# HKUST-KnowComp/DualMessagePassing

Hardware: AMD Instinct MI355X
Metric: (pattern,graph) pairs/sec DMPNN fwd+bwd hid=128 (higher is better)
Workload: dtype f32

## Files before the change

dualmessagepassing_amd/_abi.py:

```python
import ctypes

c_int = ctypes.c_int
c_i32 = ctypes.c_int32
c_i64 = ctypes.c_int64
c_u64 = ctypes.c_uint64
c_f32 = ctypes.c_float
c_double = ctypes.c_double
c_ptr = ctypes.c_void_p
c_size = ctypes.c_size_t

ABI_VERSION = 97

DMP_COLLATE_MAX_JOBS = 4
DMP_POOL_MAX_JOBS = 4
DMP_REDUCE_MAX_SEGMENTS = 16
DMP_ADAMW_MAX_SKIP = 16
DMP_ADAMW_MAX_SEGMENTS = 1024
DMP_LOOKUP_MAX_JOBS = 8
DMP_CONCAT_MAX_JOBS = 12
DMP_GEMM_MAX_JOBS = 12
DMP_GEMM_MAX_TERMS = 3
DMP_ATB_MAX_JOBS = 8
DMP_MEM_MEAN, DMP_MEM_SUM, DMP_MEM_MAX = 0, 1, 2
DMP_LRP_MAX_NEIGHBOURS = 32
# ... 197 lines not shown
    "dmp_smallk_atb_blocks": (c_i64, [c_i64]),
    "dmp_smallk_embed_cols": (c_int, [c_ptr, c_i64, c_int, c_ptr, c_i64, c_ptr, c_i64, c_int, c_int, c_ptr, c_i64, c_ptr]),
    "dmp_smallk_atb_cols_masked": (c_int, [c_ptr, c_i64, c_int, c_ptr, c_i64, c_int, c_ptr, c_i64, c_ptr, c_ptr, c_i64, c_int, c_ptr, c_ptr]),
    "dmp_smallk_atb_cols_rows": (c_int, [c_ptr, c_i64, c_int, c_ptr, c_i64, c_int, c_ptr, c_i64, c_ptr, c_ptr, c_i64, c_int, c_ptr, c_ptr]),
    "dmp_smallk_atb": (c_int, [c_ptr, c_i64, c_int, c_ptr, c_i64, c_ptr, c_i64, c_int, c_ptr, c_ptr]),
    "dmp_smallk_atb_jobs": (c_int, [_p(dmp_smallk_job), c_int, c_int, c_int, c_ptr]),
    "dmp_l0_pack_jobs": (c_int, [_p(dmp_l0_pack_job), c_int, c_ptr]),
    "dmp_count_loss": (c_int, [c_ptr, c_ptr, c_i64, c_int, c_f32, c_ptr, c_ptr, c_ptr]),
    "dmp_match_loss_workspace_words": (c_i64, [c_i64, c_i64]),
    "dmp_match_loss": (c_int, [c_ptr, c_i64, c_ptr, c_ptr, c_ptr, c_ptr, c_ptr, c_i64, c_i64, c_int, c_ptr, c_ptr, c_ptr, c_ptr, c_ptr]),
    "dmp_reduce_partials_multi": (c_int, [c_ptr, c_ptr, c_ptr, c_ptr, c_int, c_ptr]),
    "dmp_l0_pack": (c_int, [c_ptr, c_i64, c_i64, c_ptr, c_i64, c_ptr, c_i64, c_int, c_int, c_int, c_ptr, c_ptr]),
    "dmp_l0_edge_fwd_masked": (c_int, [c_ptr, c_i64, c_int, c_ptr, c_i64, c_ptr, c_i64, c_ptr, c_ptr, c_ptr, c_ptr, c_ptr, c_i64, c_int,
                                       c_f32, c_ptr, c_i64, c_ptr]),
    "dmp_l0_bwd_w_blocks": (c_i64, [c_i64]),
    "dmp_l0_node_pack_rows": (c_i64, []),
    "dmp_l0_node_fwd": (c_int, [c_ptr, c_i64, c_int, c_ptr, c_i64, c_int, c_int, c_ptr, c_i64, c_ptr, c_f32, c_ptr,
                                c_ptr, c_ptr, c_i64, c_i64, c_i64, c_i64, c_int, c_ptr, c_i64, c_ptr, c_i64, c_ptr]),
    "dmp_bn_partial_rows": (c_i64, [c_i64, c_int]),
    "dmp_bn_train_fwd": (c_int, [c_ptr, c_i64, c_i64, c_int, c_ptr, c_ptr, c_f32, c_f32, c_ptr, c_ptr, c_int, c_f32, c_ptr, c_ptr, c_ptr,
                                 c_i64, c_ptr]),
    "dmp_bn_train_bwd": (c_int, [c_ptr, c_i64, c_ptr, c_i64, c_ptr, c_i64, c_i64, c_int, c_ptr, c_int, c_f32, c_ptr, c_ptr, c_ptr, c_i64,
                                 c_ptr]),
    "dmp_bn_train_fwd_rows": (c_int, [c_ptr, c_i64, c_i64, c_ptr, c_int, c_ptr, c_ptr, c_f32, c_f32, c_ptr, c_ptr, c_int, c_f32, c_ptr, c_ptr,
                                      c_ptr, c_i64, c_ptr]),
    "dmp_bn_train_bwd_rows": (c_int, [c_ptr, c_i64, c_ptr, c_i64, c_ptr, c_i64, c_i64, c_ptr, c_int, c_ptr, c_int, c_f32, c_ptr, c_ptr, c_ptr,
                                      c_i64, c_ptr]),
    "dmp_l0_bwd_w_masked": (c_int, [c_ptr, c_i64, c_int, c_ptr, c_ptr, c_i64, c_ptr, c_i64, c_ptr, c_i64, c_int, c_ptr, c_ptr]),
    "dmp_scalar_filter_gates": (c_int, [_p(dmp_filter_job), c_int, c_i64, c_ptr, c_i64, c_ptr]),
    "dmp_csr_pair_workspace_words": (c_size, [c_i64]),
    "dmp_csr_build_pair": (c_int, [c_ptr, c_ptr, c_ptr, c_i64, c_i64, c_ptr, c_ptr, c_ptr, c_ptr, c_ptr, c_ptr, c_ptr, c_ptr, c_ptr,
                                   c_ptr, c_ptr]),
    "dmp_heads_blend": (c_int, [c_ptr, c_ptr, c_ptr, c_int, c_int, c_ptr, c_ptr]),
    "dmp_concat_pairs": (c_int, [_p(dmp_concat_job), c_int, c_ptr]),
    "dmp_table_rows": (c_int, [_p(dmp_lookup_job), c_int, c_ptr]),
    "dmp_len_masks": (c_int, [_p(dmp_mask_job), c_int, c_i64, c_ptr]),
    "dmp_pack_segments": (c_int, [c_ptr, c_ptr, c_ptr, c_int, c_int, c_ptr, c_ptr]),
    "dmp_adamw_step": (c_int, [c_ptr, c_ptr, c_ptr, c_ptr, c_ptr, c_i64, c_double, c_double, c_double, c_double,
                               c_double, c_i64, c_ptr]),
    "dmp_adamw_step_skip": (c_int, [c_ptr, c_ptr, c_ptr, c_ptr, c_ptr, c_i64, c_double, c_double, c_double, c_double,
                                    c_double, c_i64, c_ptr, c_ptr, c_int, c_ptr]),
    "dmp_adamw_step_dev": (c_int, [c_ptr, c_ptr, c_ptr, c_ptr, c_ptr, c_i64, c_ptr, c_double, c_double, c_double, c_double,
                                   c_ptr, c_ptr, c_int, c_ptr]),
    "dmp_adamw_step_segments": (c_int, [c_ptr, c_ptr, c_ptr, c_ptr, c_ptr, c_i64, c_ptr, c_ptr, c_int, c_ptr, c_ptr, c_ptr, c_double, c_double,
                                        c_double, c_double, c_ptr, c_int, c_ptr]),
    "dmp_adamw_step_guarded": (c_int, [c_ptr, c_ptr, c_ptr, c_ptr, c_ptr, c_i64, c_ptr, c_double, c_double, c_double, c_double,
                                       c_ptr, c_ptr, c_int, c_ptr, c_int, c_ptr]),
    "dmp_edge_select_build": (c_int, [c_ptr, c_ptr, c_ptr, c_ptr, c_i64, c_ptr, c_ptr, c_ptr, c_ptr]),
    "dmp_edge_select_nodes": (c_int, [c_ptr, c_ptr, c_ptr, c_ptr, c_i64, c_ptr, c_ptr, c_ptr, c_ptr]),
    "dmp_edge_fwd_fused": (c_int, [c_ptr, c_i64, c_ptr, c_i64, c_ptr, c_i64, c_i64, c_ptr, c_ptr, c_ptr, c_ptr,
                                   c_i64, c_int, c_f32, c_ptr, c_i64, c_ptr]),
    "dmp_edge_fwd_typed": (c_int, [c_ptr, c_i64, c_ptr, c_i64, c_ptr, c_i64, c_i64, c_ptr, c_ptr, c_ptr, c_ptr, c_ptr,
                                   c_ptr, c_i64, c_i64, c_int, c_f32, c_ptr, c_i64, c_ptr]),
    "dmp_bwd_z_typed_arow": (c_int, [c_ptr, c_i64, c_ptr, c_i64, c_ptr, c_i64, c_i64, c_ptr, c_i64, c_ptr, c_ptr, c_f32,
                                     c_f32, c_ptr, c_ptr, c_ptr, c_ptr, c_i64, c_i64, c_int, c_int, c_ptr, c_i64, c_ptr, c_i64, c_ptr]),
    "dmp_mask_slots": (c_int, [c_ptr, c_i64, c_ptr, c_i64, c_ptr, c_ptr]),
    "dmp_pool_relu_bwd_blocks": (c_i64, [c_i64, c_int]),
    "dmp_pool_relu_bwd": (c_int, [c_ptr, c_i64, c_ptr, c_i64, c_ptr, c_ptr, c_ptr, c_ptr, c_i64, c_i64, c_int, c_f32, c_ptr, c_i64,
                                  c_ptr, c_ptr, c_ptr]),
    "dmp_relu_bwd_gathered_colsum": (c_int, [c_ptr, c_i64, c_ptr, c_ptr, c_ptr, c_i64, c_i64, c_int, c_f32, c_ptr, c_i64, c_ptr, c_ptr]),
    "dmp_dev_set_exact_fp32": (None, [c_int]),
    "dmp_dev_get_exact_fp32": (c_int, []),
    "dmp_rel_gemm": (c_int, [c_ptr, c_i64, c_i64, c_ptr, c_i64, c_int, c_int, c_ptr, c_ptr, c_ptr, c_ptr, c_i64, c_ptr, c_i64,
                             c_int, c_ptr, c_i64, c_ptr]),
    "dmp_rel_atb_blocks": (c_i64, [c_int]),
    "dmp_rel_atb": (c_int, [c_ptr, c_i64, c_i64, c_ptr, c_i64, c_i64, c_ptr, c_ptr, c_ptr, c_ptr, c_int, c_i64, c_int, c_ptr, c_ptr]),
# ... 107 lines not shown
```

dualmessagepassing_amd/csrc/dmp_heads.hip:

```cpp
#include "dmp_common.h"

namespace dmp {
namespace {

constexpr int kThreads = 256, kRows = 16;
constexpr int kMaxHeads = DMP_HEADS_MAX;

template <int kH> struct HeadGeom {
  static constexpr int kF = 4 * kH + 4, kYS = kH + 4;
  static constexpr int kPad = kH + 4, kFPad = 4 * kH + 8;
  static constexpr int CW = kH / 16;
  static constexpr int NT = kH / 64, NKB = kH / 16;
};

__device__ __forceinline__ float4 ldg4(const float *p) { return *reinterpret_cast<const float4 *>(p); }

struct Heads {
  dmp_head_weights w[kMaxHeads];
  dmp_head_io io[kMaxHeads];
  dmp_head_grads gr[kMaxHeads];
  int B;
  float slope;
};

// ... 285 lines not shown
    if (!ok16p(io[i].ps) || !ok16p(io[i].gs) || !io[i].pl || !io[i].gl || !ok16p(io[i].F) || !ok16p(io[i].Y1S) || !io[i].y ||
        io[i].ld_ps < kH || io[i].ld_gs < kH || io[i].ld_ps % 4 || io[i].ld_gs % 4)
      return false;
  }
  return true;
}

constexpr int kLossThreads = 1024;
__global__ __launch_bounds__(kLossThreads) void count_loss_k(const float *__restrict__ pred, const float *__restrict__ target, int64_t n,
                                                             int kind, float slope, float *__restrict__ loss, float *__restrict__ dpred) {
  __shared__ float red[kLossThreads];
  const float inv_n = 1.f / (float)n;
  float acc = 0.f;
  for (int64_t i = threadIdx.x; i < n; i += kLossThreads) {
    const float p = pred[i];
    const float da = p > 0.f ? 1.f : slope;
    const float d = p * da - target[i];
    float v, g;
    if (kind == 0) { v = d * d; g = 2.f * d; }
    else if (kind == 1) { v = fabsf(d); g = d > 0.f ? 1.f : (d < 0.f ? -1.f : 0.f); }
    else { const float a = fabsf(d); v = a < 1.f ? 0.5f * d * d : a - 0.5f; g = a < 1.f ? d : (d > 0.f ? 1.f : -1.f); }
    acc += v;
    dpred[i] = g * da * inv_n;
  }
  red[threadIdx.x] = acc;
  __syncthreads();
  for (int w = kLossThreads / 2; w > 0; w >>= 1) {
    if ((int)threadIdx.x < w) red[threadIdx.x] += red[threadIdx.x + w];
    __syncthreads();
  }
  if (threadIdx.x == 0) loss[0] = red[0] * inv_n;
}

}
}

using namespace dmp;

extern "C" {

int dmp_heads_forward(const dmp_head_weights *w, const dmp_head_io *io, int num_heads, int B, int H, float slope,
                      void *stream) {
  if ((H != 128 && H != 64 && H > 0) || !slope_ok(slope)) return DMP_ERR_UNSUPPORTED;
  if (!heads_valid(w, io, num_heads, B, H)) return DMP_ERR_BAD_ARG;
  if (B == 0) return DMP_OK;
  Heads t;
  for (int i = 0; i < num_heads; ++i) { t.w[i] = w[i]; t.io[i] = io[i]; t.gr[i] = dmp_head_grads{}; }
  t.B = B; t.slope = slope;
  const dim3 grid((unsigned)((B + kRows - 1) / kRows), (unsigned)num_heads);
  if (H == 128) heads_fwd_k<128><<<grid, kThreads, 0, (hipStream_t)stream>>>(t);
  else heads_fwd_k<64><<<grid, kThreads, 0, (hipStream_t)stream>>>(t);
  return check_launch();
}

int dmp_heads_blend(const float *const *y, const float *const *gl, float *const *w, int num_heads, int B, float *out,
                    void *stream) {
  if (num_heads < 1 || num_heads > kMaxHeads || B < 0 || !y || !gl || !w) return DMP_ERR_BAD_ARG;
  if (B == 0) return DMP_OK;
  if (!out) return DMP_ERR_BAD_ARG;
  BlendArgs a;
  for (int i = 0; i < num_heads; ++i) {
    if (!y[i] || !gl[i] || !w[i]) return DMP_ERR_BAD_ARG;
    a.y[i] = y[i]; a.gl[i] = gl[i]; a.w[i] = w[i];
  }
  a.out = out; a.n = num_heads; a.B = B;
  heads_blend_k<<<(unsigned)((B + kThreads - 1) / kThreads), kThreads, 0, (hipStream_t)stream>>>(a);
// ... 10 lines not shown
        (g[i].dgs && (!ok16p(g[i].dgs) || g[i].ld_dgs % 4)) || !g[i].dWp || !g[i].dbp || !g[i].dWg || !g[i].dbg || !g[i].dW1 ||
        !g[i].db1 || !g[i].dW2 || !g[i].db2)
      return DMP_ERR_BAD_ARG;
  }
  if (B == 0) return DMP_OK;
  Heads t;
  WJobs wj;
  wj.n = 0; wj.B = B;
  int blocks = 0;
  for (int i = 0; i < num_heads; ++i) {
    t.w[i] = w[i]; t.io[i] = io[i]; t.gr[i] = g[i];
    add_wjob(wj, blocks, g[i].dY1, kH, kH, nullptr, io[i].F, kF, kF, g[i].dW1, kF, g[i].db1, 1.0f);
    add_wjob(wj, blocks, g[i].dP, kH, kH, nullptr, io[i].ps, io[i].ld_ps, kH, g[i].dWp, kH, g[i].dbp, io[i].scale_p);
    add_wjob(wj, blocks, g[i].dG, kH, kH, nullptr, io[i].gs, io[i].ld_gs, kH, g[i].dWg, kH, g[i].dbg, io[i].scale_g);
    add_wjob(wj, blocks, g[i].dy, 1, 1, g[i].dy_scale, io[i].Y1S, kYS, kYS, g[i].dW2, kYS, g[i].db2, 1.0f);
  }
  t.B = B; t.slope = slope;
  const dim3 grid((unsigned)((B + kRows - 1) / kRows), (unsigned)num_heads);
  if (H == 128) heads_bwd_rows_k<128><<<grid, kThreads, 0, (hipStream_t)stream>>>(t);
  else heads_bwd_rows_k<64><<<grid, kThreads, 0, (hipStream_t)stream>>>(t);
  int rc = check_launch();
  if (rc != DMP_OK) return rc;
  heads_bwd_w_k<<<(unsigned)blocks, kThreads, 0, (hipStream_t)stream>>>(wj);
  return check_launch();
}

int dmp_count_loss(const float *pred, const float *target, int64_t n, int kind, float neg_slope, float *loss, float *dpred, void *stream) {
  if (n < 1 || kind < 0 || kind > 2 || !pred || !target || !loss || !dpred) return DMP_ERR_BAD_ARG;
  if (n > ((int64_t)1 << 22) || !(neg_slope >= 0.f && neg_slope <= 1.f)) return DMP_ERR_UNSUPPORTED;
  count_loss_k<<<1, kLossThreads, 0, (hipStream_t)stream>>>(pred, target, n, kind, neg_slope, loss, dpred);
  return check_launch();
}

}
```

dualmessagepassing_amd/fused.py:

```python
import ctypes as _ctypes
import os as _os
import threading

import torch
from torch.autograd.function import once_differentiable

from . import _abi, _lib, gatememo, ops, side
from ._lib import check, ptr, stream_ptr


def _partials(rows, H, dev):
    lib = _lib.load()
    return torch.empty((int(lib.dmp_colsum_partial_rows(rows, H)), H), dtype=torch.float32, device=dev)


MAX_REDUCE_SEGMENTS = _abi.DMP_REDUCE_MAX_SEGMENTS


class _Deferred(threading.local):

    def __init__(self):
        self.stack = []


# ... 63 lines not shown
    lib = _lib.load()
    R, H = d_out.shape
    part = _partials(R, H, d_out.device)
    d_upd = torch.empty_like(d_out) if gate is not None else None
    with _lib.timed("scale_rows_colsum[H=%d,R=%d]", (H, R), 4 * H * R * (2 if gate is not None else 1)):
        check(lib.dmp_scale_rows_colsum(ptr(d_out), H, ptr(gate), R, H, ptr(d_upd), H, ptr(part), stream_ptr()),
              "dmp_scale_rows_colsum")
    return (d_upd if gate is not None else d_out), reduce_partials(part)


def relu_bwd_colsum_(d_h, act, out=None, slope=0.0):
    lib = _lib.load()
    R, H = d_h.shape
    part = _partials(R, H, d_h.device)
    dst = d_h if out is None else out
    ldo = dst.stride(0) if R > 1 else H
    with _lib.timed("relu_bwd_colsum[H=%d,R=%d]", (H, R), 12 * H * R):
        check(lib.dmp_relu_bwd_colsum(ptr(d_h), H, ptr(act), H, R, H, slope, ptr(dst), ldo, ptr(part), stream_ptr()),
              "dmp_relu_bwd_colsum")
    return dst, reduce_partials(part)


def relu_bwd_gathered_colsum(table, rowmap, gate, act, slope=0.0):
    lib = _lib.load()
    R, H = act.shape
    part = _partials(R, H, act.device)
    out = torch.empty((R, H), dtype=torch.float32, device=act.device)
    with _lib.timed("relu_bwd_gathered[H=%d,R=%d]", (H, R), 8 * H * R + 8 * R + 4 * H * table.size(0)):
        check(lib.dmp_relu_bwd_gathered_colsum(ptr(table), table.stride(0), ptr(rowmap), ptr(gate), ptr(act), act.stride(0), R, H,
                                               slope, ptr(out), H, ptr(part), stream_ptr()), "dmp_relu_bwd_gathered_colsum")
    return out, reduce_partials(part)


def pool_relu_bwd(table, rowmap, gate, act, pool, slope=0.0, skip_dead=False):
    lib = _lib.load()
    R, H = act.shape
    V = pool.num_chunks
    nb = int(lib.dmp_pool_relu_bwd_blocks(V, H))
    part = torch.empty((nb, H), dtype=torch.float32, device=act.device)
    kc = keep_pool_csr(pool, gate) if skip_dead else None
    vptr, vent = (pool.vptr, pool.vent) if kc is None else kc
    out = dead_rows_buffer((R, H), act.device) if kc is not None else torch.empty((R, H), dtype=torch.float32, device=act.device)
    qc = torch.empty((V, 2 * H), dtype=torch.float32, device=act.device)
    with _lib.timed("pool_relu_bwd[H=%d,R=%d]", (H, R), 8 * H * R + 12 * R + 8 * H * V):
        check(lib.dmp_pool_relu_bwd(ptr(act), act.stride(0), ptr(table), table.stride(0), ptr(rowmap), ptr(gate), ptr(vptr),
                                    ptr(vent), V, R, H, slope, ptr(out), H, ptr(qc), ptr(part), stream_ptr()), "dmp_pool_relu_bwd")
    Q = ops.seg_sum_raw(qc, pool.gptr, pool.gent, pool.num_graphs, None, False, rows_shared=False)
    return out, reduce_partials(part), Q


def keep_pool_csr(pool, gate):
    own = None if gate is None else gatememo.owner(gate)
    if not has_row_mask(own, True, True) or pool.num_chunks == 0 or gate.numel() == 0:
        return None
    return gatememo.memo(own, ("keep_pool", id(pool)), (pool,), lambda: _csr_keep(pool.vptr, pool.vent, gate, pool.num_chunks), True)


def _csr_keep_buffers(rows, entries, device):
    nscr = int(_lib.load().dmp_csr_keep_scratch_words(rows))
    ws = torch.empty(nscr + rows + 1 + entries, dtype=torch.int32, device=device)
    return ws[:nscr], ws[nscr:nscr + rows + 1], ws[nscr + rows + 1:]


def _csr_keep(csr_ptr, csr_ent, gate, rows):
    row_cnt, kptr, kent = _csr_keep_buffers(rows, csr_ent.numel(), csr_ptr.device)
    check(_lib.load().dmp_csr_keep(ptr(csr_ptr), ptr(csr_ent), ptr(gate.reshape(-1)), rows, csr_ent.numel(), ptr(row_cnt), ptr(kptr),
                                   ptr(kent), stream_ptr()), "dmp_csr_keep")
    return kptr, kent


def pool_rows(x, pool, weight=None):
    split = pool.flag8 is not None
    kc = keep_pool_csr(pool, weight) if (weight is not None and x.size(1) % 4 == 0 and x.is_contiguous()) else None
    if kc is not None:
        part = ops.seg_sum_raw(x, kc[0], kc[1], pool.num_chunks, None, split, 1.0, 1.0, rows_shared=False)
    else:
        part = ops.seg_sum_raw(x, pool.vptr, pool.vent, pool.num_chunks, weight, split, 1.0, 1.0, rows_shared=False)
    return ops.seg_sum_raw(part, pool.gptr, pool.gent, pool.num_graphs, None, False, rows_shared=False)


def pool_weight_sums(pool, weight=None):
    lib = _lib.load()
    if not getattr(pool, "rows_in_order", False):
        raise _lib.DmpError("pool_weight_sums: an index over rows in their own order")

    def build():
        halves = 2 if pool.flag8 is not None else 1
        out = torch.empty((pool.num_graphs, halves), dtype=torch.float32, device=pool.offsets.device)
        w = None if weight is None else weight.reshape(-1).contiguous()
        check(lib.dmp_pool_weight_sums(ptr(w), ptr(pool.flag8), ptr(pool.offsets), pool.num_graphs, ptr(out), stream_ptr()),
              "dmp_pool_weight_sums")
        return out

    if weight is None or weight.requires_grad:
        return build()
    return gatememo.memo(weight, "pool_weight_sums", (pool,), build)


def pool_rowmap(pool):
    m = getattr(pool, "_rowmap", None)
    if m is None:
        m = pool.seg32 if pool.flag8 is None else torch.where(pool.flag8 != 0, torch.full_like(pool.seg32, -1), pool.seg32)
        pool._rowmap = m
    return m


def bwd_g_colsum(d_y, coef, dst32):
    lib = _lib.load()
    E, H = d_y.shape
    part = _partials(E, H, d_y.device)
    d_g = torch.empty((E, 2 * H), dtype=torch.float32, device=d_y.device)
# ... 1247 lines not shown
    lib = _lib.load()
    if not 0 < len(jobs) <= _abi.DMP_GEMM_MAX_JOBS:
        raise _lib.DmpError("small_gemm_jobs: 1..%d jobs" % _abi.DMP_GEMM_MAX_JOBS)
    J = (_abi.dmp_gemm_job * len(jobs))()

    def ld(t):
        if t.dim() != 2 or t.dtype != torch.float32 or (t.size(1) > 1 and t.stride(1) != 1):
            raise _lib.DmpError("small_gemm_jobs: 2-D fp32 operands with unit inner stride")
        return t.stride(0) if t.size(0) > 1 else max(t.size(1), 1)

    keep = []
    for n, (out, terms, addend) in enumerate(jobs):
        M, N = out.shape
        if not 0 < len(terms) <= _abi.DMP_GEMM_MAX_TERMS:
            raise _lib.DmpError("small_gemm_jobs: 1..%d terms per job" % _abi.DMP_GEMM_MAX_TERMS)
        _lib.require_gpu(out, addend, *[x for tm in terms for x in (tm[0], tm[2])])
        for q, (A, ta, B, tb) in enumerate(terms):
            K = A.size(0) if ta else A.size(1)
            if (A.size(1) if ta else A.size(0)) != M or (B.size(1) if tb else B.size(0)) != K or (B.size(0) if tb else B.size(1)) != N:
                raise _lib.DmpError("small_gemm_jobs: shapes of job %d, term %d" % (n, q))
            T = J[n].term[q]
            T.A, T.lda, T.B, T.ldb, T.transA, T.transB, T.K = A.data_ptr(), ld(A), B.data_ptr(), ld(B), int(bool(ta)), int(bool(tb)), K
            keep.append((A, B))
        J[n].num_terms, J[n].M, J[n].N, J[n].C, J[n].ldc = len(terms), M, N, out.data_ptr(), ld(out)
        if addend is not None:
            if addend.shape != out.shape:
                raise _lib.DmpError("small_gemm_jobs: addend shape")
            J[n].C0, J[n].ldc0 = addend.data_ptr(), ld(addend)
    check(lib.dmp_small_gemm_jobs(J, len(jobs), stream_ptr()), "dmp_small_gemm_jobs")


class _LayerCall:
    __slots__ = ("index", "coef", "residual", "H", "N", "slope", "inner", "v_gate", "e_gate", "Bn", "bn", "Wx", "Wes", "be",
                 "nW2", "nb2", "eW2", "eb2", "WesT", "nW2t", "eW2t", "l0", "W0", "WV0", "nd", "vpool", "epool")

    def __init__(self, **facts):
        for name in self.__slots__:
            setattr(self, name, facts[name])


def _kept_nodes(index, H, v_gate, l0):
    side.wait("nodes")
    return node_rows(index, v_gate, H) if kept_node_path(index, H, v_gate, l0) else None


def _xn_buffer(c, device):
    return dead_rows_buffer((c.N, c.H), device) if (c.inner & 1) else torch.zeros((c.N, c.H), dtype=torch.float32, device=device)


def _l0_param_products(c, node_pass, device):
    l0, W0, WV0, H, Bn, Wx = c.l0, c.W0, c.WV0, c.H, c.Bn, c.Wx
    K0, TK = l0.K, W0.size(0)
    M0 = torch.empty((TK, 2 * H), dtype=torch.float32, device=device)
    jobs = [(M0, [(W0, False, c.Wes, False)], None)]
    WP = WB = MV = None
    if node_pass:
        VK = l0.VK
        WP = torch.zeros((TK // K0, L0_NODE_MAX_COLS, 3 * H), dtype=torch.float32, device=device)
        for t in range(TK // K0):
            WVt = WV0 if WV0.size(0) == VK else WV0[t * VK:(t + 1) * VK]
            jobs += [(WP[t, :VK], [(WVt, False, Wx, False)], None),
                     (WP[t, VK:VK + K0, :H], [(W0[t * K0:(t + 1) * K0], False, Bn[:H], False)], None),
                     (WP[t, VK + K0:VK + 2 * K0, :H], [(W0[t * K0:(t + 1) * K0], False, Bn[H:], False)], None)]
    else:
        WB = torch.empty((2, TK, H), dtype=torch.float32, device=device)
        jobs += [(WB[0], [(W0, False, Bn[:H], False)], None), (WB[1], [(W0, False, Bn[H:], False)], None)]
        if l0.venc is not None:
# ... 137 lines not shown
        tiles = _edge_out_tiles(c, z, dead, False)
        if tiles is not None:
            H1e = dead_rows_buffer((z.size(0), H), z.device)
            zn = out_fwd_typed(H1e, c.eW2t, c.eb2, z, tiles,
                               first=dict(z=z, Wes=c.Wes, P=P, ldp=ldp, bias=c.be, coef=c.coef, index=c.index, slope=c.slope, sel=sel))
            return H1e, zn
    if typed_ok(c.index, H):
        return edge_fwd_typed(z, c.Wes, P, ldp, c.be, c.coef, c.index, c.slope, dead_gate=dead_gate, sel=sel), None
    G = z @ c.Wes
    H1e = edge_combine_raw(G, 2 * H, P, ldp, c.be, c.coef, c.index, H, relu=True, slope=c.slope)
    del G
    if sums_only:
        return H1e, None
    Oe = torch.addmm(c.eb2, H1e, c.eW2.t())
    return H1e, gate_residual(z if c.residual else None, Oe, c.e_gate)


def _edge_out(c, z, H1e):
    l0 = c.l0
    _, dead = _dead_edge_rows_of(c)
    side.wait("tiles")
    codes = _residual_from_codes(c, H1e)
    tiles = _edge_out_tiles(c, H1e, dead, codes)
    if tiles is None:
        return out_fwd_mfma(H1e, c.eW2, c.eb2, c.e_gate, l0_rows(l0, c.W0, z) if c.residual else None, c.eW2t, dead_rows=dead)
    walk = ascending_tiles(c.e_gate) or tiles
    if codes:
        return out_fwd_typed_codes(H1e, c.eW2t, c.eb2, l0.enc, l0.K, c.W0[-l0.K:], walk, prev=l0.z_head, row0=l0.z_head.size(0))
    return out_fwd_typed(H1e, c.eW2t, c.eb2, l0_rows(l0, c.W0, z) if c.residual else None, walk)


def _pooled_outputs(c, z, xn, zn, H1e, sums_only):
    H, epool, e_gate, eW2, eb2 = c.H, c.epool, c.e_gate, c.eW2, c.eb2
    vs = pool_rows(xn, c.vpool) if c.vpool is not None else None
    if not sums_only:
        return vs, (pool_rows(zn, epool) if epool is not None else None), None
    halves = 2 if epool.flag8 is not None else 1
    G_ = epool.num_graphs
    Q = pool_rows(H1e, epool, e_gate).view(G_ * halves, H)
    gcnt = pool_weight_sums(epool, e_gate)
    cnt = gcnt.view(G_ * halves, 1)
    zs = pool_rows(z, epool, e_gate if zero_rows_gate(e_gate) else None).view(G_ * halves, H) if c.residual else None
    if Q.is_contiguous() and eW2.is_contiguous() and Q.size(0) <= SMALL_GEMM_MAX_ROWS:
        es = torch.empty((G_ * halves, H), dtype=torch.float32, device=Q.device)
        small_gemm_jobs([(es, [(Q, False, eW2, True), (cnt, False, eb2.view(1, H), False)], zs)])
    else:
        es = torch.addmm(zs, Q, eW2.t()) if c.residual else Q @ eW2.t()
        es.addcmul_(cnt, eb2.view(1, H))
    return vs, es.view(G_, halves * H)[:, :H], gcnt


def _grad_seeds(c, x, z, H1e, dxn, dzn, dvs, des, typed):
    H = c.H
    lazy = None
    if dvs is not None:
        exp = ops.gather_rows_raw(dvs.contiguous(), c.vpool.seg32)
        dxn = exp if dxn is None else dxn + exp
    if des is not None:
        ep = c.epool
        if dzn is None and typed and H1e.size(0) > 0 and des.size(1) == H:
            lazy = (des.contiguous(), pool_rowmap(ep), ep)
        else:
            if ep.flag8 is not None and des.size(1) == H:
                des = torch.cat([des, torch.zeros_like(des)], dim=1)
            exp = (ops.gather_select_raw(des.contiguous(), ep.seg32, ep.flag8, H, None, 1.0, 1.0) if ep.flag8 is not None
                   else ops.gather_rows_raw(des.contiguous(), ep.seg32))
            dzn = exp if dzn is None else dzn + exp
    if dxn is None:
        dxn = torch.zeros_like(x)
    if dzn is None and lazy is None:
        dzn = torch.zeros_like(z)
    return dxn.contiguous(), (dzn.contiguous() if dzn is not None else None), lazy


def l0_tables_full(l0, tables, W0):
    return all(r[1] > r[0] and n[1] > n[0] for _, r, n in tables) and len(tables) * l0.K == W0.size(0)


def l0_codes_buffer(l0, tables, W0, residual, H, device):
    return (torch.empty if l0_tables_full(l0, tables, W0) else torch.zeros)((W0.size(0), (3 if residual else 2) * H),
                                                                           dtype=torch.float32, device=device)


def l0_codes_block(c, tables, device, walked):
    if not h1w_codes_ok(c.l0, tables or (), walked):
        return None
    t, rows, _ = tables[-1]
    XX, K0 = l0_codes_buffer(c.l0, tables, c.W0, c.residual, c.H, device), c.l0.K
    return XX, dict(enc=c.l0.enc, K=K0, coef_e=c.index.edge_select(c.coef)[2], rows=rows, residual=c.residual, out=XX[t * K0:(t + 1) * K0])


def _edge_out_bwd_lazy(c, H1e, lazy, gcnt):
    H, e_gate = c.H, c.e_gate
    T, emap, ep = lazy
    if H % 4 == 0 and H <= 256:
        skip = c.l0 is None and c.nd is not None and USE_PLAIN_ATB and dead_edge_rows(c.index, H, e_gate, c.coef)
        dG, dbe, Q = pool_relu_bwd(T @ c.eW2, emap, e_gate, H1e, ep, c.slope, skip_dead=skip)
        Q = Q[:, :H]
    else:
        dG, dbe = relu_bwd_gathered_colsum(T @ c.eW2, emap, e_gate, H1e, c.slope)
        Q = pool_rows(H1e, ep, e_gate)[:, :H]
    dW2e = T.t() @ Q
    if gcnt is None:
        gcnt = pool_weight_sums(ep, e_gate)
    return dG, dbe, dW2e, gcnt[:, 0] @ T


def _edge_out_bwd_typed(c, tables, H1e, dzn):
    ix, coef, H, slope, e_gate, eW2 = c.index, c.coef, c.H, c.slope, c.e_gate, c.eW2
    l0_XX = None
    if binary_gate_mask(e_gate) is not None:
        skip = USE_MASKED_SUMS and dead_h1_rows(ix, H, e_gate) and (c.l0 is None or c.l0.enc_mask is not None)
        lt = live_tiles(ix, coef, e_gate) if skip else None
        if lt is not None and h1w_ok(dzn, H1e, H):
            l0_XX = l0_codes_block(c, tables, dzn.device, "kept")
            dG, dbe, db2e, dW2e = bwd_h1_w(dzn, eW2, H1e, ascending_tiles(e_gate) or lt, slope, codes=l0_XX and l0_XX[1])[:4]
        elif lt is not None:
            dG, dbe, db2e = bwd_h1_typed(dzn, eW2, H1e, ascending_tiles(e_gate) or lt, slope)
            dW2e = atb_typed(dzn, H1e, coef, ix, gate=e_gate, plain=True)
        else:
            dG, dbe, db2e = bwd_h1_mfma(dzn, eW2, H1e, coef, ix, both_halves=False, gate=e_gate, slope=slope, rows_colsum=True,
                                        skip_dead_stores=skip)
            dW2e = atb_rows(dzn, H1e, e_gate, colsum=False)[0]
        return dG, dbe, dW2e, db2e, l0_XX
    it = identity_tiles(dzn.size(0), dzn.device) if (e_gate is None and h1w_ok(dzn, H1e, H)) else None
    if it is not None:
        l0_XX = l0_codes_block(c, tables, dzn.device, "all")
# ... 224 lines not shown
    return bwd_z_typed(dG, dG.stride(0), Wes, dS, base, coef, ix, c.WesT, base_map=base_map, gate=e_gate, dead_rows=dead_dz,
                       dst=dst_m), dWes


def _l0_final_products(c, XX, Xn, Yn, dWx):
    H, W0, WV0, Bn, Wx, dev = c.H, c.W0, c.WV0, c.Bn, c.Wx, XX.device
    dWes = torch.empty((H, 2 * H), dtype=torch.float32, device=dev)
    dBn = torch.empty((2 * H, H), dtype=torch.float32, device=dev)
    dW0 = torch.empty((W0.size(0), H), dtype=torch.float32, device=dev)
    dWV0 = None
    jobs = [(dWes, [(W0, True, XX[:, :2 * H], False)], None),
            (dBn[:H], [(W0, True, Xn[0], False)], None), (dBn[H:], [(W0, True, Xn[1], False)], None),
            (dW0, [(XX[:, :2 * H], False, c.Wes, True), (Xn[0], False, Bn[:H], True), (Xn[1], False, Bn[H:], True)],
             XX[:, 2 * H:] if c.residual else None)]
    if Yn is not None:
        dWx = torch.empty((H, 3 * H), dtype=torch.float32, device=dev)
        dWV0 = torch.empty((WV0.size(0), H), dtype=torch.float32, device=dev)
        for b3 in range(3):
            jobs.append((dWx[:, b3 * H:(b3 + 1) * H], [(WV0, True, Yn[b3], False)], None))
        jobs.append((dWV0, [(Yn[b3], False, Wx[:, b3 * H:(b3 + 1) * H], True) for b3 in range(3)], Yn[3] if c.residual else None))
    small_gemm_jobs(jobs)
    return dBn, dWx, dWes, dW0, dWV0


class _FusedDMPLayer(torch.autograd.Function):

    @staticmethod
    def forward(ctx, index, coef, residual, x, z, v_gate, e_gate, Bn, bn, Wx, Wes, be, nW2, nb2, eW2, eb2,
                WesT=None, nW2t=None, eW2t=None, slope=0.0, vpool=None, epool=None, l0=None, W0=None, WV0=None, edge_rows=True,
                inner=0):
        _lib.require_gpu(x, z)
        H = Bn.size(1)
        x, z = x.contiguous(), z.contiguous()
        c = _LayerCall(index=index, coef=coef, residual=residual, H=H, N=index.num_nodes, slope=slope, inner=int(inner),
                       v_gate=v_gate, e_gate=e_gate, Bn=Bn.contiguous(), bn=bn, Wx=Wx.contiguous(), Wes=Wes.contiguous(), be=be,
                       nW2=nW2, nb2=nb2, eW2=eW2, eb2=eb2, WesT=WesT, nW2t=nW2t, eW2t=eW2t, l0=l0,
                       W0=None if l0 is None else W0.detach(), WV0=None if (l0 is None or WV0 is None) else WV0.detach(),
                       nd=_kept_nodes(index, H, v_gate, l0), vpool=vpool, epool=epool)
        S = S0 = M0 = tables = xn = chain_panels = None
        if l0 is not None:
            S0, M0, tables, H1n, P, ldp = _node_first_codes(c, x, z)
        else:
            S, H1n, P, ldp, xn, chain_panels = _node_first_rows(c, x, z)
        if xn is None:
            xn = _node_out(c, x, H1n)
        sums_only = epool is not None and not edge_rows
        if l0 is not None:
            H1e, zn = _edge_first_codes(c, z, M0, tables, P, ldp, sums_only)
        else:
            H1e, zn = _edge_first_rows(c, z, P, ldp, sums_only)
        if zn is None and not sums_only:
            zn = _edge_out(c, z, H1e)
        ctx.call, ctx.chain_panels, ctx.l0_S0, ctx.l0_tables, ctx.gcnt = c, chain_panels, S0, tables, None
        ctx.save_for_backward(x, z if l0 is None else None, S, H1n, H1e)
        if vpool is None and epool is None:
            return xn, zn
        ctx.set_materialize_grads(False)
        vs, es, ctx.gcnt = _pooled_outputs(c, z, xn, zn, H1e, sums_only)
        return xn, zn, vs, es

    @staticmethod
    @once_differentiable
    def backward(ctx, dxn, dzn, dvs=None, des=None):
        x, z, S, H1n, H1e = ctx.saved_tensors
        c, tables = ctx.call, ctx.l0_tables
        typed = typed_ok(c.index, c.H)
        want_dx, want_dz = ctx.needs_input_grad[3], ctx.needs_input_grad[4]
        dxn, dzn, lazy = _grad_seeds(c, x, z, H1e, dxn, dzn, dvs, des, typed)
        dz = dW0 = dWV0 = None
        with deferred_reductions():
            dG, dbe, dW2e, db2e, l0_XX = _edge_out_bwd(c, tables, H1e, dzn, lazy, ctx.gcnt, typed)
            dXP = _endpoint_sums(c, dG, typed, x.device)
            if c.l0 is not None:
                XX = _l0_edge_code_products(c, tables, dG, dzn, l0_XX)
                dbn, dWx, dW2n, db2n, Xn, Yn, dx = _node_bwd_codes(c, tables, ctx.l0_S0, x, H1n, dxn, dXP, want_dx)
            else:
                dWes = _edge_first_wgrad(c, z, dG, typed, want_dz)
                dBn, dbn, dWx, dW2n, db2n, dS, dx = _node_bwd_rows(c, ctx.chain_panels, x, S, H1n, dxn, dXP, want_dx)
                if want_dz:
# ... 48 lines not shown
```

include/dmp_hip.h:

```cpp
#ifndef DMP_HIP_H
#define DMP_HIP_H

#include <stddef.h>
#include <stdint.h>

#ifdef __cplusplus
extern "C" {
#endif

#define DMP_OK 0
#define DMP_ERR_BAD_ARG (-1)
#define DMP_ERR_UNSUPPORTED (-2)
#define DMP_ERR_HIP (-3)

#define DMP_ABI_VERSION 97
int dmp_abi_version(void);
const char *dmp_last_hip_error(void);


size_t dmp_csr_workspace_words(int64_t num_nodes, int64_t num_edges);

int dmp_csr_build(const int64_t *key, const uint8_t *flag, int64_t num_edges,
                  int64_t num_nodes, int32_t *rowptr, int32_t *ent,
                  int32_t *key32, int64_t *degree, int32_t *status,
// ... 399 lines not shown
} dmp_gemm_term;
typedef struct {
  dmp_gemm_term term[DMP_GEMM_MAX_TERMS];
  const float *C0; int64_t ldc0; float *C; int64_t ldc; int32_t num_terms, M, N, pad;
} dmp_gemm_job;
int dmp_small_gemm_jobs(const dmp_gemm_job *jobs, int num_jobs, void *stream);


#define DMP_HEADS_MAX 2
typedef struct { const float *Wp, *bp, *Wg, *bg, *W1, *b1, *W2, *b2; } dmp_head_weights;
typedef struct {
  const float *ps; int64_t ld_ps; const float *gs; int64_t ld_gs; const float *pl, *gl; float scale_p, scale_g;
  float *F, *Y1S, *y;
} dmp_head_io;
typedef struct {
  const float *dy, *dy_scale; float *dY1, *dP, *dG; float *dps; int64_t ld_dps; float *dgs; int64_t ld_dgs;
  float *dWp, *dbp, *dWg, *dbg, *dW1, *db1, *dW2, *db2;
} dmp_head_grads;
int dmp_heads_forward(const dmp_head_weights *w, const dmp_head_io *io, int num_heads, int B, int H,
                      float slope, void *stream);

int dmp_count_loss(const float *pred, const float *target, int64_t n, int kind, float neg_slope, float *loss, float *dpred, void *stream);
int dmp_heads_backward(const dmp_head_weights *w, const dmp_head_io *io, const dmp_head_grads *g,
                       int num_heads, int B, int H, float slope, void *stream);

int64_t dmp_match_loss_workspace_words(int64_t B, int64_t Lc);
int dmp_match_loss(const float *pred, int64_t ldp, const int64_t *w, const uint8_t *mask, const float *pred_c,
                   const float *pair_w, const float *coef, int64_t B, int64_t Lc, int kind, float *terms, float *dpred,
                   float *dpred_c, void *workspace, void *stream);

int dmp_heads_blend(const float *const *y, const float *const *gl, float *const *w, int num_heads, int B, float *out,
                    void *stream);



int dmp_edge_select_build(const int32_t *src, const int32_t *dst, const uint8_t *flag,
                          const float *coef, int64_t num_edges, int32_t *selA, int32_t *selB,
                          float *coefE, void *stream);
int dmp_edge_select_nodes(const int32_t *src, const int32_t *dst, const uint8_t *flag, const uint32_t *nodemask,
                          int64_t num_edges, int32_t *selA, int32_t *selB, int32_t *dstM, void *stream);

int dmp_edge_fwd_fused(const float *Z, int64_t ldz, const float *W, int64_t ldw,
                       const float *P, int64_t ldp, int64_t num_nodes, const float *bias,
                       const int32_t *selA, const int32_t *selB, const float *coefE,
                       int64_t num_edges, int H, float slope, float *H1, int64_t ldh, void *stream);


int64_t dmp_mfma_partial_rows_h(int64_t num_edges, int H);

int dmp_row_mask_bits(const float *gate, int64_t E, uint32_t *mask, void *stream);
int dmp_row_mask_rows(const float *X, int64_t ldx, int K, int64_t R, uint32_t *mask, void *stream);

int dmp_out_fwd_fused_rows(const float *Hin, int64_t ldh, const float *W2, int64_t ldw, const float *bias,
                           const float *gate, const uint32_t *rowmask, int dead_rows, const float *R, int64_t ldr, int64_t E, int H,
                           int w_in_out, float *out, int64_t ldo, void *stream);
int dmp_bwd_h1_fused_rows(const float *dO, int64_t ldo, const float *W2, int64_t ldw, const float *H1, int64_t ldh,
                          const float *coefE, const float *gate, const uint32_t *rowmask, int skip_dead_stores, int64_t E, int H,
                          float slope, float *dG, int64_t ldg, float *partial, float *partial_rows, void *stream);

int64_t dmp_typed_partial_rows(int64_t tiles_bound, int H);
typedef struct {
  const float *Hin; int64_t ldh;
  const float *W2; int64_t ldw; int w_in_out;
  const float *bias;
  const float *R; int64_t ldr;
  const float *R2; int64_t ldr2;
// ... 208 lines not shown
```

Before: 504,500.

## Pool edge hidden rows before the output GEMM via linearity, with fused pool kernels

```diff
diff --git a/dualmessagepassing_amd/_abi.py b/dualmessagepassing_amd/_abi.py
--- a/dualmessagepassing_amd/_abi.py
+++ b/dualmessagepassing_amd/_abi.py
@@ -253,6 +253,11 @@
     "dmp_csr_build_pair": (c_int, [c_ptr, c_ptr, c_ptr, c_i64, c_i64, c_ptr, c_ptr, c_ptr, c_ptr, c_ptr, c_ptr, c_ptr, c_ptr, c_ptr,
                                    c_ptr, c_ptr]),
     "dmp_heads_blend": (c_int, [c_ptr, c_ptr, c_ptr, c_int, c_int, c_ptr, c_ptr]),
+    "dmp_pool_out": (c_int, [c_ptr, c_ptr, c_i64, c_int, c_ptr, c_ptr, c_i64, c_ptr, c_ptr, c_ptr, c_ptr, c_i64, c_ptr, c_ptr, c_i64,
+                             c_int, c_ptr, c_ptr, c_ptr, c_ptr]),
+    "dmp_rows_gemm": (c_int, [c_ptr, c_i64, c_i64, c_int, c_ptr, c_int, c_ptr, c_i64, c_ptr]),
+    "dmp_pool_wgrad_blocks": (c_i64, [c_i64]),
+    "dmp_pool_wgrad": (c_int, [c_ptr, c_i64, c_i64, c_int, c_ptr, c_ptr, c_i64, c_ptr, c_i64, c_ptr, c_int, c_ptr, c_ptr, c_ptr]),
     "dmp_concat_pairs": (c_int, [_p(dmp_concat_job), c_int, c_ptr]),
     "dmp_table_rows": (c_int, [_p(dmp_lookup_job), c_int, c_ptr]),
     "dmp_len_masks": (c_int, [_p(dmp_mask_job), c_int, c_i64, c_ptr]),
diff --git a/dualmessagepassing_amd/csrc/dmp_heads.hip b/dualmessagepassing_amd/csrc/dmp_heads.hip
--- a/dualmessagepassing_amd/csrc/dmp_heads.hip
+++ b/dualmessagepassing_amd/csrc/dmp_heads.hip
@@ -341,6 +341,188 @@
   if (threadIdx.x == 0) loss[0] = red[0] * inv_n;
 }
 
+constexpr int kWgGraphs = 32;
+
+template <int CW>
+__device__ __forceinline__ void chunk_sum(float (&acc)[CW], float (&acc2)[CW], const float *part, const float *part2, int64_t ld,
+                                          int64_t V, const int32_t *gptr, const int32_t *gent, int64_t g, int col) {
+  constexpr int U = 4;
+#pragma unroll
+  for (int e = 0; e < CW; ++e) { acc[e] = 0.f; acc2[e] = 0.f; }
+  const int beg = gptr[g], end = gptr[g + 1];
+  for (int p = beg; p < end; p += U) {
+    float4 v[U][CW / 4], v2[U][CW / 4];
+    bool ok[U];
+#pragma unroll
+    for (int u = 0; u < U; ++u) {
+      ok[u] = false;
+      if (p + u < end) {
+        const int64_t ch = gent[p + u] >> 1;
+        ok[u] = ch >= 0 && ch < V;
+        if (ok[u]) {
+#pragma unroll
+          for (int q = 0; q < CW / 4; ++q) v[u][q] = ldg4(part + ch * ld + col + 4 * q);
+          if (part2) {
+#pragma unroll
+            for (int q = 0; q < CW / 4; ++q) v2[u][q] = ldg4(part2 + ch * ld + col + 4 * q);
+          }
+        }
+      }
+    }
+#pragma unroll
+    for (int u = 0; u < U; ++u) {
+      if (ok[u]) {
+#pragma unroll
+        for (int q = 0; q < CW / 4; ++q) {
+          acc[4 * q] += v[u][q].x; acc[4 * q + 1] += v[u][q].y; acc[4 * q + 2] += v[u][q].z; acc[4 * q + 3] += v[u][q].w;
+        }
+        if (part2) {
+#pragma unroll
+          for (int q = 0; q < CW / 4; ++q) {
+            acc2[4 * q] += v2[u][q].x; acc2[4 * q + 1] += v2[u][q].y; acc2[4 * q + 2] += v2[u][q].z; acc2[4 * q + 3] += v2[u][q].w;
+          }
+        }
+      }
+    }
+  }
+}
+
+struct PoolOut {
+  const float *partH, *partZ, *partX, *gcnt, *W2, *b2;
+  const int32_t *gptr, *gent, *ngptr, *ngent;
+  float *es, *vs, *Q;
+  int64_t ldh, V, Vn;
+  int G, Gn, halves, eblocks;
+};
+
+template <int kH>
+__global__ __launch_bounds__(kThreads) void pool_out_k(const PoolOut a) {
+  constexpr int kPad = HeadGeom<kH>::kPad, CW = HeadGeom<kH>::CW;
+  __shared__ float As[kRows * kPad];
+  __shared__ float Ws[16 * kPad];
+  const int tid = threadIdx.x, r = tid >> 4, cg = tid & 15, col = cg * CW;
+  float q[CW], zs[CW];
+  if ((int)blockIdx.x >= a.eblocks) {
+    const int64_t g = (int64_t)((int)blockIdx.x - a.eblocks) * kRows + r;
+    if (g >= a.Gn) return;
+    chunk_sum<CW>(q, zs, a.partX, nullptr, kH, a.Vn, a.ngptr, a.ngent, g, col);
+    store_cw<CW>(a.vs + g * kH + col, q);
+    return;
+  }
+  const int64_t g = (int64_t)blockIdx.x * kRows + r;
+  const bool live = g < a.G;
+#pragma unroll
+  for (int e = 0; e < CW; ++e) { q[e] = 0.f; zs[e] = 0.f; }
+  if (live) chunk_sum<CW>(q, zs, a.partH, a.partZ, a.ldh, a.V, a.gptr, a.gent, g, col);
+  const float cnt = (live && a.b2) ? a.gcnt[g * a.halves] : 0.f;
+  store_cw<CW>(&As[r * kPad + col], q);
+  if (live && a.Q) store_cw<CW>(a.Q + g * kH + col, q);
+  float es[CW];
+#pragma unroll
+  for (int e = 0; e < CW; ++e) es[e] = 0.f;
+  gemm_h<kH>(es, As, kPad, a.W2, kH, 1, 0, Ws, tid, cg);
+  if (!live) return;
+  if (a.partZ) {
+#pragma unroll
+    for (int e = 0; e < CW; ++e) es[e] = zs[e] + es[e];
+  }
+  if (a.b2) {
+#pragma unroll
+    for (int e = 0; e < CW; ++e) es[e] += cnt * a.b2[col + e];
+  }
+  store_cw<CW>(a.es + g * kH + col, es);
+}
+
+template <int kH>
+__global__ __launch_bounds__(kThreads) void rows_gemm_k(const float *__restrict__ A, int64_t lda, int rows, const float *__restrict__ W, int wT,
+                                                        float *__restrict__ out, int64_t ldo) {
+  constexpr int kPad = HeadGeom<kH>::kPad, CW = HeadGeom<kH>::CW;
+  __shared__ float As[kRows * kPad];
+  __shared__ float Ws[16 * kPad];
+  const int tid = threadIdx.x, r = tid >> 4, cg = tid & 15, i0 = (int)blockIdx.x * kRows;
+  float acc[CW];
+#pragma unroll
+  for (int e = 0; e < CW; ++e) acc[e] = 0.f;
+  stage_rows<kH>(As, A, lda, i0, rows, tid);
+  gemm_h<kH>(acc, As, kPad, W, kH, wT, 0, Ws, tid, cg);
+  if (i0 + r < rows) store_cw<CW>(out + (int64_t)(i0 + r) * ldo + cg * CW, acc);
+}
+
+struct PoolWgrad {
+  const float *qc, *T, *gcnt;
+  const int32_t *gptr, *gent;
+  float *part, *Q;
+  int64_t ldq, ldt, V;
+  int G, halves;
+};
+
+template <int kH>
+__global__ __launch_bounds__(kThreads) void pool_wgrad_k(const PoolWgrad a) {
+  typedef float f32x4 __attribute__((ext_vector_type(4)));
+  constexpr int CW = kH / 8, JT = kH / 64, KT = kH / 16;
+  constexpr int kWPad = kH + 16;
+  __shared__ float Ts[kWgGraphs * kWPad];
+  __shared__ float Qs[kWgGraphs * kWPad];
+  __shared__ float Cs[kWgGraphs];
+  const int tid = threadIdx.x, r = tid >> 3, cg = tid & 7, col = cg * CW;
+  const int lane = tid & 63, wave = tid >> 6, m = lane & 15, kq = lane >> 4;
+  const int64_t g = (int64_t)blockIdx.x * kWgGraphs + r;
+  const bool live = g < a.G;
+  float q[CW], tv[CW], unused[CW];
+#pragma unroll
+  for (int e = 0; e < CW; ++e) { q[e] = 0.f; tv[e] = 0.f; }
+  if (live) {
+#pragma unroll
+    for (int v = 0; v < CW / 4; ++v) {
+      const float4 t4 = ldg4(a.T + g * a.ldt + col + 4 * v);
+      tv[4 * v] = t4.x; tv[4 * v + 1] = t4.y; tv[4 * v + 2] = t4.z; tv[4 * v + 3] = t4.w;
+    }
+    if (cg == 0) Cs[r] = a.gcnt[g * a.halves];
+    chunk_sum<CW>(q, unused, a.qc, nullptr, a.ldq, a.V, a.gptr, a.gent, g, col);
+    if (a.Q) store_cw<CW>(a.Q + g * kH + col, q);
+  } else if (cg == 0) {
+    Cs[r] = 0.f;
+  }
+  store_cw<CW>(&Qs[r * kWPad + col], q);
+  store_cw<CW>(&Ts[r * kWPad + col], tv);
+  __syncthreads();
+  f32x4 d[JT][KT];
+#pragma unroll
+  for (int jt = 0; jt < JT; ++jt)
+#pragma unroll
+    for (int kt = 0; kt < KT; ++kt) d[jt][kt] = f32x4{0.f, 0.f, 0.f, 0.f};
+#pragma unroll
+  for (int s = 0; s < kWgGraphs / 4; ++s) {
+    const int row = (4 * s + kq) * kWPad;
+    float av[JT];
+#pragma unroll
+    for (int jt = 0; jt < JT; ++jt) av[jt] = Ts[row + (wave * JT + jt) * 16 + m];
+#pragma unroll
+    for (int kt = 0; kt < KT; ++kt) {
+      const float b = Qs[row + kt * 16 + m];
+#pragma unroll
+      for (int jt = 0; jt < JT; ++jt) d[jt][kt] = __builtin_amdgcn_mfma_f32_16x16x4f32(av[jt], b, d[jt][kt], 0, 0, 0);
+    }
+  }
+  float *P = a.part + (int64_t)blockIdx.x * (kH * kH + kH);
+#pragma unroll
+  for (int jt = 0; jt < JT; ++jt)
+#pragma unroll
+    for (int kt = 0; kt < KT; ++kt)
+#pragma unroll
+      for (int i = 0; i < 4; ++i) P[((wave * JT + jt) * 16 + 4 * kq + i) * kH + kt * 16 + m] = d[jt][kt][i];
+  if (tid < kH) {
+    float db = 0.f;
+#pragma unroll
+    for (int rr = 0; rr < kWgGraphs; ++rr) db += Cs[rr] * Ts[rr * kWPad + tid];
+    P[kH * kH + tid] = db;
+  }
+}
+
+inline bool pool_csr_ok(const int32_t *gptr, const int32_t *gent, int64_t V, int64_t G) {
+  return gptr && (gent || V == 0) && V >= 0 && G >= 0 && G < ((int64_t)1 << 24) && V < ((int64_t)1 << 30);
+}
+
 }
 }
 
@@ -417,4 +599,54 @@
   return check_launch();
 }
 
-}
+int dmp_pool_out(const float *partH, const float *partZ, int64_t V, int halves, const int32_t *gptr, const int32_t *gent, int64_t G,
+                 const float *gcnt, const float *W2, const float *b2, const float *partX, int64_t Vn, const int32_t *ngptr,
+                 const int32_t *ngent, int64_t Gn, int H, float *es, float *vs, float *Q, void *stream) {
+  if (H != 128 && H != 64) return DMP_ERR_UNSUPPORTED;
+  if ((halves != 1 && halves != 2) || !pool_csr_ok(gptr, gent, V, G)) return DMP_ERR_BAD_ARG;
+  if (G > 0 && (((V > 0 || partH) && !ok16p(partH)) || (partZ && !ok16p(partZ)) || !ok16p(W2) || (b2 && (!ok16p(b2) || !gcnt)) || !ok16p(es) || (Q && !ok16p(Q))))
+    return DMP_ERR_BAD_ARG;
+  if (!partX) Gn = 0;
+  if (partX && (!pool_csr_ok(ngptr, ngent, Vn, Gn) || (Gn > 0 && (!ok16p(partX) || !ok16p(vs))))) return DMP_ERR_BAD_ARG;
+  if (G == 0 && Gn == 0) return DMP_OK;
+  PoolOut a;
+  a.partH = partH; a.partZ = partZ; a.partX = partX; a.gcnt = gcnt; a.W2 = W2; a.b2 = b2;
+  a.gptr = gptr; a.gent = gent; a.ngptr = ngptr; a.ngent = ngent; a.es = es; a.vs = vs; a.Q = Q;
+  a.ldh = (int64_t)halves * H; a.V = V; a.Vn = Vn; a.G = (int)G; a.Gn = (int)Gn; a.halves = halves;
+  a.eblocks = (int)((G + kRows - 1) / kRows);
+  const unsigned grid = (unsigned)(a.eblocks + (Gn + kRows - 1) / kRows);
+  if (H == 128) pool_out_k<128><<<grid, kThreads, 0, (hipStream_t)stream>>>(a);
+  else pool_out_k<64><<<grid, kThreads, 0, (hipStream_t)stream>>>(a);
+  return check_launch();
+}
+
+int dmp_rows_gemm(const float *A, int64_t lda, int64_t rows, int H, const float *W, int w_out_in, float *out, int64_t ldo,
+                  void *stream) {
+  if (H != 128 && H != 64) return DMP_ERR_UNSUPPORTED;
+  if (rows < 0 || rows >= ((int64_t)1 << 30) || lda < H || ldo < H || lda % 4 || ldo % 4) return DMP_ERR_BAD_ARG;
+  if (rows == 0) return DMP_OK;
+  if (!ok16p(A) || !ok16p(W) || !ok16p(out)) return DMP_ERR_BAD_ARG;
+  const unsigned grid = (unsigned)((rows + kRows - 1) / kRows);
+  if (H == 128) rows_gemm_k<128><<<grid, kThreads, 0, (hipStream_t)stream>>>(A, lda, (int)rows, W, w_out_in ? 1 : 0, out, ldo);
+  else rows_gemm_k<64><<<grid, kThreads, 0, (hipStream_t)stream>>>(A, lda, (int)rows, W, w_out_in ? 1 : 0, out, ldo);
+  return check_launch();
+}
+
+int64_t dmp_pool_wgrad_blocks(int64_t G) { return G > 0 ? (G + kWgGraphs - 1) / kWgGraphs : 0; }
+
+int dmp_pool_wgrad(const float *qc, int64_t ldq, int64_t V, int halves, const int32_t *gptr, const int32_t *gent, int64_t G,
+                   const float *T, int64_t ldt, const float *gcnt, int H, float *partial, float *Q, void *stream) {
+  if (H != 128 && H != 64) return DMP_ERR_UNSUPPORTED;
+  if ((halves != 1 && halves != 2) || !pool_csr_ok(gptr, gent, V, G) || ldt < H || ldt % 4 || ldq < H || ldq % 4) return DMP_ERR_BAD_ARG;
+  if (G == 0) return DMP_OK;
+  if (((V > 0 || qc) && !ok16p(qc)) || !ok16p(T) || !gcnt || !ok16p(partial) || (Q && !ok16p(Q))) return DMP_ERR_BAD_ARG;
+  PoolWgrad a;
+  a.qc = qc; a.T = T; a.gcnt = gcnt; a.gptr = gptr; a.gent = gent; a.part = partial; a.Q = Q;
+  a.ldq = ldq; a.ldt = ldt; a.V = V; a.G = (int)G; a.halves = halves;
+  const unsigned grid = (unsigned)dmp_pool_wgrad_blocks(G);
+  if (H == 128) pool_wgrad_k<128><<<grid, kThreads, 0, (hipStream_t)stream>>>(a);
+  else pool_wgrad_k<64><<<grid, kThreads, 0, (hipStream_t)stream>>>(a);
+  return check_launch();
+}
+
+}
diff --git a/dualmessagepassing_amd/fused.py b/dualmessagepassing_amd/fused.py
--- a/dualmessagepassing_amd/fused.py
+++ b/dualmessagepassing_amd/fused.py
@@ -119,7 +119,7 @@
     return out, reduce_partials(part)
 
 
-def pool_relu_bwd(table, rowmap, gate, act, pool, slope=0.0, skip_dead=False):
+def pool_relu_bwd(table, rowmap, gate, act, pool, slope=0.0, skip_dead=False, chunk_sums=False):
     lib = _lib.load()
     R, H = act.shape
     V = pool.num_chunks
@@ -132,6 +132,8 @@
     with _lib.timed("pool_relu_bwd[H=%d,R=%d]", (H, R), 8 * H * R + 12 * R + 8 * H * V):
         check(lib.dmp_pool_relu_bwd(ptr(act), act.stride(0), ptr(table), table.stride(0), ptr(rowmap), ptr(gate), ptr(vptr),
                                     ptr(vent), V, R, H, slope, ptr(out), H, ptr(qc), ptr(part), stream_ptr()), "dmp_pool_relu_bwd")
+    if chunk_sums:
+        return out, reduce_partials(part), qc
     Q = ops.seg_sum_raw(qc, pool.gptr, pool.gent, pool.num_graphs, None, False, rows_shared=False)
     return out, reduce_partials(part), Q
 
@@ -157,13 +159,73 @@
 
 
 def pool_rows(x, pool, weight=None):
+    return ops.seg_sum_raw(pool_chunk_sums(x, pool, weight), pool.gptr, pool.gent, pool.num_graphs, None, False, rows_shared=False)
+
+
+def pool_chunk_sums(x, pool, weight=None):
     split = pool.flag8 is not None
     kc = keep_pool_csr(pool, weight) if (weight is not None and x.size(1) % 4 == 0 and x.is_contiguous()) else None
     if kc is not None:
-        part = ops.seg_sum_raw(x, kc[0], kc[1], pool.num_chunks, None, split, 1.0, 1.0, rows_shared=False)
-    else:
-        part = ops.seg_sum_raw(x, pool.vptr, pool.vent, pool.num_chunks, weight, split, 1.0, 1.0, rows_shared=False)
-    return ops.seg_sum_raw(part, pool.gptr, pool.gent, pool.num_graphs, None, False, rows_shared=False)
+        return ops.seg_sum_raw(x, kc[0], kc[1], pool.num_chunks, None, split, 1.0, 1.0, rows_shared=False)
+    return ops.seg_sum_raw(x, pool.vptr, pool.vent, pool.num_chunks, weight, split, 1.0, 1.0, rows_shared=False)
+
+
+USE_POOL_ALGEBRA = True
+POOL_ALGEBRA_WIDTHS = (64, 128)
+
+
+def _aligned(*tensors):
+    return all(t is None or (t.dtype == torch.float32 and t.is_contiguous() and t.data_ptr() % 16 == 0) for t in tensors)
+
+
+def pool_algebra_ok(index, H, epool, eW2, eb2):
+    return bool(USE_POOL_ALGEBRA and H in POOL_ALGEBRA_WIDTHS and getattr(epool, "rows_in_order", False) and epool.num_graphs > 0
+                and index.num_edges > 0 and typed_ok(index, H) and eb2 is not None and _aligned(eW2, eb2))
+
+
+def pool_out(partH, partZ, pool, gcnt, W2, b2, partX=None, vpool=None, want_q=False):
+    lib = _lib.load()
+    H, G, V = W2.size(0), pool.num_graphs, pool.num_chunks
+    halves = partH.size(1) // H
+    dev = partH.device
+    es = torch.empty((G, H), dtype=torch.float32, device=dev)
+    Q = torch.empty((G, H), dtype=torch.float32, device=dev) if want_q else None
+    Gn, Vn = (vpool.num_graphs, vpool.num_chunks) if partX is not None else (0, 0)
+    vs = torch.empty((Gn, H), dtype=torch.float32, device=dev) if partX is not None else None
+    nbytes = 4 * H * (V * (2 if partZ is not None else 1) + H + G + Vn + Gn) + 4 * (V + Vn + 2 * G + Gn)
+    with _lib.timed("pool_out[H=%d,G=%d]", (H, G), nbytes):
+        check(lib.dmp_pool_out(ptr(partH), ptr(partZ), V, halves, ptr(pool.gptr), ptr(pool.gent), G, ptr(gcnt), ptr(W2), ptr(b2),
+                               ptr(partX), Vn, ptr(vpool.gptr) if partX is not None else None,
+                               ptr(vpool.gent) if partX is not None else None, Gn, H, ptr(es), ptr(vs), ptr(Q), stream_ptr()),
+              "dmp_pool_out")
+    return (es, vs, Q) if want_q else (es, vs)
+
+
+def rows_gemm(a, W, w_out_in):
+    lib = _lib.load()
+    R, H = a.shape
+    out = torch.empty((R, H), dtype=torch.float32, device=a.device)
+    with _lib.timed("rows_gemm[H=%d,R=%d]", (H, R), 4 * H * (2 * R + H)):
+        check(lib.dmp_rows_gemm(ptr(a), a.stride(0) if R > 1 else H, R, H, ptr(W), int(bool(w_out_in)), ptr(out), H, stream_ptr()),
+              "dmp_rows_gemm")
+    return out
+
+
+def pool_wgrad(qc, pool, T, gcnt, want_q=False):
+    lib = _lib.load()
+    G, H = T.shape
+    V = pool.num_chunks
+    nb = int(lib.dmp_pool_wgrad_blocks(G))
+    if nb == 0:
+        z = torch.zeros(H * H + H, dtype=torch.float32, device=T.device)
+        return (z[:H * H].view(H, H), z[H * H:]) + ((torch.empty((0, H), dtype=torch.float32, device=T.device),) if want_q else ())
+    part = torch.empty((nb, H * H + H), dtype=torch.float32, device=T.device)
+    Q = torch.empty((G, H), dtype=torch.float32, device=T.device) if want_q else None
+    with _lib.timed("pool_wgrad[H=%d,G=%d]", (H, G), 4 * H * (V + G) + 4 * (V + 2 * G) + 4 * nb * (H * H + H)):
+        check(lib.dmp_pool_wgrad(ptr(qc), qc.size(1), V, gcnt.size(1), ptr(pool.gptr), ptr(pool.gent), G, ptr(T), T.stride(0) if G > 1 else H, ptr(gcnt),
+                                 H, ptr(part), ptr(Q), stream_ptr()), "dmp_pool_wgrad")
+    out = reduce_partials(part)
+    return (out[:H * H].view(H, H), out[H * H:]) + ((Q,) if want_q else ())
 
 
 def pool_weight_sums(pool, weight=None):
@@ -1477,7 +1539,7 @@
 
 class _LayerCall:
     __slots__ = ("index", "coef", "residual", "H", "N", "slope", "inner", "v_gate", "e_gate", "Bn", "bn", "Wx", "Wes", "be",
-                 "nW2", "nb2", "eW2", "eb2", "WesT", "nW2t", "eW2t", "l0", "W0", "WV0", "nd", "vpool", "epool")
+                 "nW2", "nb2", "eW2", "eb2", "WesT", "nW2t", "eW2t", "l0", "W0", "WV0", "nd", "vpool", "epool", "poolalg")
 
     def __init__(self, **facts):
         for name in self.__slots__:
@@ -1681,6 +1743,16 @@
 
 def _pooled_outputs(c, z, xn, zn, H1e, sums_only):
     H, epool, e_gate, eW2, eb2 = c.H, c.epool, c.e_gate, c.eW2, c.eb2
+    if c.poolalg:
+        vp = c.vpool if (c.vpool is not None and c.vpool.flag8 is None) else None
+        partX = pool_chunk_sums(xn, vp) if vp is not None else None
+        partH = pool_chunk_sums(H1e, epool, e_gate)
+        gcnt = pool_weight_sums(epool, e_gate)
+        partZ = pool_chunk_sums(z, epool, e_gate if zero_rows_gate(e_gate) else None) if c.residual else None
+        es, vs = pool_out(partH, partZ, epool, gcnt, eW2, eb2, partX, vp)
+        if vp is None and c.vpool is not None:
+            vs = pool_rows(xn, c.vpool)
+        return vs, es, gcnt
     vs = pool_rows(xn, c.vpool) if c.vpool is not None else None
     if not sums_only:
         return vs, (pool_rows(zn, epool) if epool is not None else None), None
@@ -1742,6 +1814,14 @@
 def _edge_out_bwd_lazy(c, H1e, lazy, gcnt):
     H, e_gate = c.H, c.e_gate
     T, emap, ep = lazy
+    if c.poolalg:
+        T = T if _aligned(T) else T.clone(memory_format=torch.contiguous_format)
+        skip = c.l0 is None and c.nd is not None and USE_PLAIN_ATB and dead_edge_rows(c.index, H, e_gate, c.coef)
+        dG, dbe, qc = pool_relu_bwd(rows_gemm(T, c.eW2, False), emap, e_gate, H1e, ep, c.slope, skip_dead=skip, chunk_sums=True)
+        if gcnt is None:
+            gcnt = pool_weight_sums(ep, e_gate)
+        dW2e, db2e = pool_wgrad(qc, ep, T, gcnt)
+        return dG, dbe, dW2e, db2e
     if H % 4 == 0 and H <= 256:
         skip = c.l0 is None and c.nd is not None and USE_PLAIN_ATB and dead_edge_rows(c.index, H, e_gate, c.coef)
         dG, dbe, Q = pool_relu_bwd(T @ c.eW2, emap, e_gate, H1e, ep, c.slope, skip_dead=skip)
@@ -2032,11 +2112,13 @@
         _lib.require_gpu(x, z)
         H = Bn.size(1)
         x, z = x.contiguous(), z.contiguous()
+        sums_only = epool is not None and not edge_rows
         c = _LayerCall(index=index, coef=coef, residual=residual, H=H, N=index.num_nodes, slope=slope, inner=int(inner),
                        v_gate=v_gate, e_gate=e_gate, Bn=Bn.contiguous(), bn=bn, Wx=Wx.contiguous(), Wes=Wes.contiguous(), be=be,
                        nW2=nW2, nb2=nb2, eW2=eW2, eb2=eb2, WesT=WesT, nW2t=nW2t, eW2t=eW2t, l0=l0,
                        W0=None if l0 is None else W0.detach(), WV0=None if (l0 is None or WV0 is None) else WV0.detach(),
-                       nd=_kept_nodes(index, H, v_gate, l0), vpool=vpool, epool=epool)
+                       nd=_kept_nodes(index, H, v_gate, l0), vpool=vpool, epool=epool,
+                       poolalg=sums_only and pool_algebra_ok(index, H, epool, eW2, eb2))
         S = S0 = M0 = tables = xn = chain_panels = None
         if l0 is not None:
             S0, M0, tables, H1n, P, ldp = _node_first_codes(c, x, z)
@@ -2044,7 +2126,6 @@
             S, H1n, P, ldp, xn, chain_panels = _node_first_rows(c, x, z)
         if xn is None:
             xn = _node_out(c, x, H1n)
-        sums_only = epool is not None and not edge_rows
         if l0 is not None:
             H1e, zn = _edge_first_codes(c, z, M0, tables, P, ldp, sums_only)
         else:
diff --git a/include/dmp_hip.h b/include/dmp_hip.h
--- a/include/dmp_hip.h
+++ b/include/dmp_hip.h
@@ -455,6 +455,15 @@
 int dmp_heads_blend(const float *const *y, const float *const *gl, float *const *w, int num_heads, int B, float *out,
                     void *stream);
 
+int dmp_pool_out(const float *partH, const float *partZ, int64_t V, int halves, const int32_t *gptr, const int32_t *gent, int64_t G,
+                 const float *gcnt, const float *W2, const float *b2, const float *partX, int64_t Vn, const int32_t *ngptr,
+                 const int32_t *ngent, int64_t Gn, int H, float *es, float *vs, float *Q, void *stream);
+int dmp_rows_gemm(const float *A, int64_t lda, int64_t rows, int H, const float *W, int w_out_in, float *out, int64_t ldo,
+                  void *stream);
+int64_t dmp_pool_wgrad_blocks(int64_t G);
+int dmp_pool_wgrad(const float *qc, int64_t ldq, int64_t V, int halves, const int32_t *gptr, const int32_t *gent, int64_t G,
+                   const float *T, int64_t ldt, const float *gcnt, int H, float *partial, float *Q, void *stream);
+
 
 
 int dmp_edge_select_build(const int32_t *src, const int32_t *dst, const uint8_t *flag,
```

Result: faster. 517,400 (median of 6 runs) (+2.6%).
